# m4rch1n0/vqvae

Hardware: AMD Instinct MI355X
Metric: latents/sec through geodesic kNN+APSP+K-medoids (higher is better)
Workload: dtype f64-exact(u32 fixed point)

## Files before the change

include/geo_hip.h:

```cpp
#ifndef GEO_HIP_H
#define GEO_HIP_H

#include <stddef.h>
#include <stdint.h>

#ifdef __cplusplus
extern "C" {
#endif

#define GEO_OK 0
#define GEO_E_ARG (-1)
#define GEO_E_WORKSPACE (-2)
#define GEO_E_HIP (-3)
#define GEO_E_NOCONV (-4)

int geo_version(void);
const char *geo_last_error(void);

int geo_set_option(const char *name, int32_t value);

size_t geo_sssp_workspace_bytes(int32_t n, int64_t nnz, int32_t n_sources);

int geo_sssp_multi(const int32_t *indptr, const int32_t *indices, const float *weights,
                   int32_t n, int64_t nnz, const int32_t *sources, int32_t n_sources,
// ... 139 lines not shown
#define GEO_JVP_MID_PIPE 0
#define GEO_JVP_MID_PIPE_DEDUP 1
#define GEO_JVP_MID_ALL 2
#define GEO_JVP_MID_ALL_TANGENT 3
#define GEO_JVP_MID_CHUNK 4
#define GEO_JVP_BACK_MFMA 0
#define GEO_JVP_BACK_PER_NODE 1
#define GEO_JVP_BACK_DEDUP 2
#define GEO_JVP_BACK_VALU 3
#define GEO_JVP_PLAN_FRONT(p) ((p) & 3)
#define GEO_JVP_PLAN_DMAX(p) (16 << (((p) >> 2) & 3))
#define GEO_JVP_PLAN_MID(p) (((p) >> 4) & 15)
#define GEO_JVP_PLAN_BACK(p) (((p) >> 8) & 15)
#define GEO_JVP_PER_NODE 0x1000
#define GEO_JVP_NODE_JACOBIAN 0x2000
#define GEO_JVP_DEDUP 0x4000
#define GEO_JVP_FRONT_ONCE 0x8000
#define GEO_JVP_PLAN_PASSES(p) ((p) >> 16)
int geo_jvp_plan(const geo_decoder_desc *dec, int64_t n_nodes, int64_t n_edges, int32_t batch_size, int32_t graph_edges,
                 size_t ws_bytes);
int geo_jvp_plan_part(const geo_decoder_desc *dec, int64_t n_nodes, int64_t n_edges, int64_t build_edges, int32_t batch_size,
                      int32_t graph_edges, size_t ws_bytes);
int geo_jvp_head_stream(const geo_decoder_desc *dec, int64_t n_nodes, int64_t n_edges, int32_t batch_size, int32_t graph_edges);

int geo_decoder_jvp_pairs(const geo_decoder_desc *dec, const float *z_start, const float *z_end,
                          int64_t n_edges, int32_t batch_size, float *len_out,
                          void *ws, size_t ws_bytes, void *stream);


typedef struct geo_vanilla_decoder_desc {
    int32_t latent_dim;
    int32_t c1, c2;
    int32_t out_channels;
    int32_t out_size;
    const float *At;
    const float *c;
    const float *w2p;
    const float *scale2;
    const float *shift2;
    const float *w3p;
    const float *b3;
} geo_vanilla_decoder_desc;

size_t geo_vanilla_jvp_workspace_bytes(const geo_vanilla_decoder_desc *dec, int64_t n_edges);
size_t geo_vanilla_jvp_edges_workspace_bytes(const geo_vanilla_decoder_desc *dec, int64_t n_nodes, int64_t n_edges);
int geo_vanilla_jvp_pairs(const geo_vanilla_decoder_desc *dec, const float *z_start, const float *z_end, int64_t n_edges,
// ... 155 lines not shown
```

vqvae_amd/_lib.py:

```python
import ctypes
import os

import torch

_HERE = os.path.dirname(os.path.abspath(__file__))
LIB_PATH = os.path.join(_HERE, "libgeo_hip.so")

c_p = ctypes.c_void_p
i32, i64, sz = ctypes.c_int32, ctypes.c_int64, ctypes.c_size_t


class DecoderDesc(ctypes.Structure):
    _fields_ = ([(n, i32) for n in ("latent_dim", "c0", "c1", "c2", "out_channels", "out_size", "norm",
                                    "bn_train", "groups1", "groups2")]
                + [("eps", ctypes.c_float)]
                + [(n, c_p) for n in ("w_in", "b_in", "w1", "b1", "g1", "be1", "rm1", "rv1",
                                      "w2", "b2", "g2", "be2", "rm2", "rv2", "w3", "b3")]
                + [("update_running", i32), ("momentum", ctypes.c_float)])


class VanillaDecoderDesc(ctypes.Structure):
    _fields_ = ([(n, i32) for n in ("latent_dim", "c1", "c2", "out_channels", "out_size")]
                + [(n, c_p) for n in ("At", "c", "w2p", "scale2", "shift2", "w3p", "b3")])

# ... 55 lines not shown
    "geo_knn_last_path": (ctypes.c_int, []),
    "geo_knn_thresholds": (ctypes.c_int, [c_p, i64, i32, i32, i32, i64, i64, i32, c_p, c_p, sz, c_p]),
    "geo_nearest_foreign_workspace_bytes": (sz, [i64, i32]),
    "geo_nearest_foreign": (ctypes.c_int, [c_p, i64, i32, i32, c_p, c_p, i64, c_p, c_p, c_p, sz, c_p]),
    "geo_bridge_components_workspace_bytes": (sz, [i64, i32, i32]),
    "geo_bridge_components": (ctypes.c_int, [c_p, i64, i32, i32, c_p, i32, c_p, c_p, c_p, c_p, sz, c_p]),
    "geo_csr_insert_workspace_bytes": (sz, [i32, i64]),
    "geo_csr_insert_count": (ctypes.c_int, [c_p, c_p, i32, c_p, c_p, c_p, i64, c_p, c_p, c_p, sz, c_p]),
    "geo_csr_insert_fill": (ctypes.c_int, [c_p, c_p, c_p, i32, i64, c_p, c_p, c_p, c_p, sz, c_p]),
    "geo_symmetrize_workspace_bytes": (sz, [i32, i32]),
    "geo_symmetrize_count": (ctypes.c_int, [c_p, c_p, i32, i32, i32, c_p, c_p, c_p, sz, c_p]),
    "geo_symmetrize_fill": (ctypes.c_int, [c_p, c_p, i32, i32, i32, c_p, c_p, c_p, c_p, sz, c_p]),
    "geo_upper_edges_count": (ctypes.c_int, [c_p, c_p, i32, c_p, c_p, c_p, sz, c_p]),
    "geo_upper_edges_fill": (ctypes.c_int, [c_p, c_p, i32, c_p, c_p, c_p, c_p, c_p]),
    "geo_cc_workspace_bytes": (sz, [i32]),
    "geo_connected_components": (ctypes.c_int, [c_p, c_p, i32, c_p, c_p, c_p, sz, c_p]),
    "geo_csr_compact_workspace_bytes": (sz, [i32]),
    "geo_csr_compact_count": (ctypes.c_int, [c_p, c_p, c_p, i32, c_p, i32, c_p, c_p, c_p, c_p, c_p, sz, c_p]),
    "geo_csr_compact_fill": (ctypes.c_int, [c_p, c_p, c_p, i32, c_p, i32, c_p, c_p, c_p, c_p, c_p]),
    "geo_jvp_workspace_bytes": (sz, [ctypes.POINTER(DecoderDesc), i64, i32]),
    "geo_jvp_edges_workspace_bytes": (sz, [ctypes.POINTER(DecoderDesc), i64, i64, i32]),
    "geo_jvp_plan": (ctypes.c_int, [ctypes.POINTER(DecoderDesc), i64, i64, i32, i32, sz]),
    "geo_jvp_head_stream": (ctypes.c_int, [ctypes.POINTER(DecoderDesc), i64, i64, i32, i32]),
    "geo_decoder_jvp_edges": (ctypes.c_int, [ctypes.POINTER(DecoderDesc), c_p, i64, c_p, c_p, i64, i32, c_p, c_p, sz, c_p]),
    "geo_jvp_edges_part_workspace_bytes": (sz, [ctypes.POINTER(DecoderDesc), i64, i64, i64, i32]),
    "geo_jvp_plan_part": (ctypes.c_int, [ctypes.POINTER(DecoderDesc), i64, i64, i64, i32, i32, sz]),
    "geo_decoder_jvp_edges_part": (ctypes.c_int, [ctypes.POINTER(DecoderDesc), c_p, i64, c_p, c_p, i64, i64, i32, c_p, c_p, sz,
                                                  c_p]),
    "geo_decoder_jvp_pairs": (ctypes.c_int, [ctypes.POINTER(DecoderDesc), c_p, c_p, i64, i32, c_p, c_p, sz, c_p]),
    "geo_vanilla_jvp_workspace_bytes": (sz, [ctypes.POINTER(VanillaDecoderDesc), i64]),
    "geo_vanilla_jvp_edges_workspace_bytes": (sz, [ctypes.POINTER(VanillaDecoderDesc), i64, i64]),
    "geo_vanilla_jvp_pairs": (ctypes.c_int, [ctypes.POINTER(VanillaDecoderDesc), c_p, c_p, i64, i32, c_p, c_p, sz, c_p]),
    "geo_vanilla_jvp_edges": (ctypes.c_int, [ctypes.POINTER(VanillaDecoderDesc), c_p, i64, c_p, c_p, i64, i32, c_p, c_p, sz, c_p]),
    "geo_vanilla_decode_workspace_bytes": (sz, [ctypes.POINTER(VanillaDecoderDesc), i64]),
    "geo_vanilla_decode": (ctypes.c_int, [ctypes.POINTER(VanillaDecoderDesc), c_p, c_p, i64, c_p, c_p, sz, c_p]),
    "geo_spatial_decode_workspace_bytes": (sz, [ctypes.POINTER(SpatialImageDecoderDesc), i64]),
    "geo_spatial_decode": (ctypes.c_int, [ctypes.POINTER(SpatialImageDecoderDesc), c_p, c_p, c_p, i64, c_p, c_p, sz, c_p]),
    "geo_image_encode_workspace_bytes": (sz, [ctypes.POINTER(ImageEncoderDesc), i64]),
    "geo_image_encode": (ctypes.c_int, [ctypes.POINTER(ImageEncoderDesc), c_p, i64, c_p, c_p, c_p, sz, c_p]),
    "geo_lpips_alex_workspace_bytes": (sz, [i64]),
    "geo_lpips_alex": (ctypes.c_int, [ctypes.POINTER(LPIPSAlexDesc), c_p, c_p, i64, c_p, c_p, c_p, sz, c_p]),
    "geo_gather_edge_weights":(ctypes.c_int, [c_p, c_p, i64, c_p, c_p]),
    "geo_prior_sample_workspace_bytes": (sz, [ctypes.POINTER(PriorDesc), i32, i32]),
    "geo_prior_sample": (ctypes.c_int, [ctypes.POINTER(PriorDesc), c_p, i32, i32, c_p, c_p, ctypes.c_float, i32, c_p, c_p, i32,
                                        c_p, sz, c_p]),
    "geo_kmeans_workspace_bytes": (sz, [i64, i32, i32, i32, i32]),
# ... 67 lines not shown
```

vqvae_amd/csrc/common.hip:

```cpp
#include "geo_common.h"

#include <cstdlib>
#include <cstring>

namespace geo {

namespace {
struct OptionName { const char *name, *env; int Options::*field; };
const OptionName kOptionNames[] = {
    {"sssp_sb", "GEO_SSSP_SB", &Options::sssp_sb},
    {"sssp_act", "GEO_SSSP_ACT", &Options::sssp_act},
    {"sssp_sparse_div", "GEO_SSSP_SPARSE_DIV", &Options::sssp_sparse_div},
    {"sssp_map_div", "GEO_SSSP_MAP_DIV", &Options::sssp_map_div},
    {"sssp_group", "GEO_SSSP_GROUP", &Options::sssp_group},
    {"sssp_grouped_cap", "GEO_SSSP_GROUPED_CAP", &Options::sssp_grouped_cap},
    {"sssp_trace", "GEO_SSSP_TRACE", &Options::sssp_trace},
    {"sssp_u32", "GEO_SSSP_U32", &Options::sssp_u32},
    {"sssp_push", "GEO_SSSP_PUSH", &Options::sssp_push},
    {"sssp_order", "GEO_SSSP_ORDER", &Options::sssp_order},
    {"sssp_delta", "GEO_SSSP_DELTA", &Options::sssp_delta},
    {"sssp_push_blocks", "GEO_SSSP_PUSH_BLOCKS", &Options::sssp_push_blocks},
    {"knn_filter", "GEO_KNN_FILTER", &Options::knn_filter},
    {"kpp_grid", "GEO_KPP_GRID", &Options::kpp_grid},
    {"kpp_profile", "GEO_KPP_PROFILE", &Options::kpp_profile},
    {"jvp_mid", "GEO_JVP_MID", &Options::jvp_mid},
    {"jvp_back_valu", "GEO_JVP_BACK_VALU", &Options::jvp_back_valu},
    {"jvp_front_valu", "GEO_JVP_FRONT_VALU", &Options::jvp_front_valu},
    {"jvp_per_node", "GEO_JVP_PER_NODE", &Options::jvp_per_node},
    {"jvp_node_jacobian", "GEO_JVP_NODE_JACOBIAN", &Options::jvp_node_jacobian},
    {"jvp_start_dedup", "GEO_JVP_START_DEDUP", &Options::jvp_start_dedup},
    {"jvp_front_once", "GEO_JVP_FRONT_ONCE", &Options::jvp_front_once},
    {"jvp_head_stream", "GEO_JVP_HEAD_STREAM", &Options::jvp_head_stream},
};
Options from_environment() {
    Options o;
    for (const OptionName &e : kOptionNames) {
        const char *v = getenv(e.env);
        if (!v) continue;
        if (e.field == &Options::jvp_mid) o.jvp_mid = v[0] == 'c' ? 2 : (v[0] == 'a' ? 3 : atoi(v));
        else o.*(e.field) = atoi(v);
    }
    return o;
}
}

Options &options() {
    static Options o = from_environment();
    return o;
}

static thread_local char g_err[512] = "";

void set_error(const char *fmt, ...) {
    va_list ap;
    va_start(ap, fmt);
// ... 87 lines not shown
    int rc = scan_rec(sums, offs, t, ar, s);
    if (rc != GEO_OK) return rc;
    scan_add_kernel<<<dim3((unsigned)t), dim3(SCAN_THREADS), 0, s>>>(out, offs, n, t);
    GEO_LAUNCH_CHECK();
    return GEO_OK;
}

int exclusive_scan_i32(const int32_t *in, int32_t *out, int64_t n, void *tmp, size_t tmp_bytes,
                       int64_t *total_host, hipStream_t stream) {
    Arena ar(tmp, tmp_bytes);
    int rc = scan_rec(in, out, n, ar, stream);
    if (rc != GEO_OK) return rc;
    if (total_host) {
        int32_t tot = 0;
        GEO_HIP_CHECK(hipMemcpyAsync(&tot, out + n, sizeof(int32_t), hipMemcpyDeviceToHost, stream));
        GEO_HIP_CHECK(hipStreamSynchronize(stream));
        *total_host = tot;
    }
    return GEO_OK;
}

}

extern "C" int geo_version(void) { return 114; }
extern "C" const char *geo_last_error(void) { return geo::g_err; }

extern "C" int geo_set_option(const char *name, int32_t value) {
    if (name)
        for (const geo::OptionName &e : geo::kOptionNames)
            if (strcmp(name, e.name) == 0) {
                geo::options().*(e.field) = value;
                return GEO_OK;
            }
    geo::set_error("geo_set_option: unknown option '%s'", name ? name : "(null)");
    return GEO_E_ARG;
}
```

vqvae_amd/csrc/geo_common.h:

```cpp
#pragma once
#include <hip/hip_runtime.h>

#include <cstdarg>
#include <cstdint>
#include <cstdio>

#include "geo_hip.h"

namespace geo {

void set_error(const char *fmt, ...);

#define GEO_HIP_CHECK(expr)                                                                      \
    do {                                                                                         \
        hipError_t _e = (expr);                                                                  \
        if (_e != hipSuccess) {                                                                  \
            geo::set_error("%s failed: %s (%s:%d)", #expr, hipGetErrorString(_e), __FILE__, __LINE__); \
            return GEO_E_HIP;                                                                    \
        }                                                                                        \
    } while (0)

#define GEO_REQUIRE(cond, ...)              \
    do {                                    \
        if (!(cond)) {                      \
            geo::set_error(__VA_ARGS__);    \
            return GEO_E_ARG;               \
        }                                   \
    } while (0)

#define GEO_LAUNCH_CHECK() GEO_HIP_CHECK(hipGetLastError())

struct Options {
    int sssp_sb = -1, sssp_act = 1, sssp_sparse_div = -1, sssp_map_div = -1, sssp_group = 1, sssp_grouped_cap = 256,
        sssp_trace = 0, sssp_u32 = 1, sssp_push = 1 ,
        sssp_delta = 8 , sssp_order = 0 , sssp_push_blocks = 64, knn_filter = 1, kpp_grid = 256, kpp_profile = 0, jvp_mid = 0 ,
        jvp_back_valu = 0, jvp_front_valu = 0, jvp_per_node = 1 ,
        jvp_node_jacobian = 1 ,
        jvp_start_dedup = 1 ,
        jvp_front_once = 1 ,
        jvp_head_stream = 1 ;
};
Options &options();

static inline size_t align_up(size_t x, size_t a = 256) { return (x + a - 1) / a * a; }

struct Arena {
    char *base;
    size_t size, off;
    Arena(void *p, size_t n) : base(static_cast<char *>(p)), size(n), off(0) {}
    template <typename T>
    T *take(size_t count) {
        size_t bytes = align_up(count * sizeof(T));
        if (off + bytes > size) return nullptr;
        T *r = reinterpret_cast<T *>(base + off);
        off += bytes;
        return r;
    }
};

static inline int64_t shrink_pass(int64_t items) { return items > 64 ? items - items / 8 : items - 1; }

static inline size_t pass_bytes(const size_t *per_item, int nb, int64_t items) {
    size_t bytes = 0;
// ... 41 lines not shown
```

vqvae_amd/csrc/jvp.hip:

```cpp
#include "geo_common.h"

#include <cmath>
#include <cstdlib>
#include <type_traits>
#include <vector>

namespace {

constexpr int TS = 32;
constexpr int NC = 128;
constexpr int MAX_BLOCKS = 4;
constexpr int FRONT_MAX_N1 = 1024;
constexpr int BACK_TS = 8;

typedef float f32x16 __attribute__((ext_vector_type(16)));
typedef __bf16 bf16x8 __attribute__((ext_vector_type(8)));
typedef unsigned short u16x8 __attribute__((ext_vector_type(8)));

struct Shape {
    int d, c0, c1, c2, co, s_out, pad3, p_out;
    int n1, n2;
    int opix_per_chunk, n_chunks;
};

// ... 1136 lines not shown
        const int64_t e = e_base + (int64_t)chunk * batch + within;
        const bool valid = within < slots_per_group && within < batch && e < n_edges;
        const bool head = valid && start_run_head(src, e, within);
        const unsigned long long m = __ballot(head);
        const int below = __popcll(m & ((1ull << lane) - 1ull));
        if (lane == 0) wsum[wave] = __popcll(m);
        __syncthreads();
        int before = carry, total = carry;
        for (int w = 0; w < 4; ++w) { if (w < wave) before += wsum[w]; total += wsum[w]; }
        const int k = before + below + (head ? 1 : 0) - 1;
        if (within < slots_per_group) {
            row_map[g0 + within] = (int32_t)(g0 + (valid ? k : 0));
            if (head) rep[g0 + k] = (int32_t)(g0 + within);
        }
        carry = total;
        __syncthreads();
    }
    if (threadIdx.x == 0) { carry_s = carry; n_compact[chunk] = carry; }
    __syncthreads();
    const int cnt = carry_s, padded = (cnt + TS - 1) / TS * TS;
    for (int k = cnt + (int)threadIdx.x; k < padded; k += 256) rep[g0 + k] = (int32_t)g0;
}

template <bool TT, bool ONCE = false>
__global__ __launch_bounds__(512, 2) void mid_start_kernel(const float *__restrict__ pre1, const float *__restrict__ tpre1,
                                                          const NormConst *__restrict__ consts1, int tiles_per_group,
                                                          const unsigned short *__restrict__ B3, const float *__restrict__ b2,
                                                          float *__restrict__ pre2, float *__restrict__ tpre2,
                                                          double *__restrict__ partial2, const int32_t *__restrict__ row_map,
                                                          const int32_t *__restrict__ rep, const int32_t *__restrict__ n_compact,
                                                          int64_t e_base, int64_t n_edges, int batch) {
    constexpr int C1 = 128, LDK = C1 + 8, KS = C1 / 16, NL = 4, c2 = 64, n1 = 4 * C1, n2 = 16 * c2;
    typedef float f32x2 __attribute__((ext_vector_type(2)));
    __shared__ __attribute__((aligned(16))) unsigned short A3[2][3][2][TS][LDK];
    const int chunk = blockIdx.y, group = 2 * chunk;
    const int ncomp = TT ? 0 : n_compact[chunk];
    auto run = [&](int item) {
    const int lt0 = 2 * item;
    const bool live1 = TT ? lt0 + 1 < tiles_per_group : (lt0 + 1) * TS < ncomp;
    const int tile0 = group * tiles_per_group + lt0, tile1 = live1 ? tile0 + 1 : tile0;
    const int lane = threadIdx.x & 63, wave = __builtin_amdgcn_readfirstlane((int)(threadIdx.x >> 6));
    const int wq = wave & 3, wg = wave >> 2;
    const int r = lane & 31, h = lane >> 5;
    f32x16 accp[NL], acct[NL];
#pragma unroll
    for (int lc = 0; lc < NL; ++lc)
#pragma unroll
        for (int i = 0; i < 16; ++i) { accp[lc][i] = 0.f; acct[lc][i] = 0.f; }

    const int k0p = 2 * lane, s0p = 4 * wave;
    const NormConst *kp = consts1 + (size_t)group * C1 + k0p;
    const NormConst kA = kp[0], kB = kp[1];
    static_assert(TT || !ONCE, "ONCE selects where the tangent launch reads");
    size_t xrow[2][4];
    const size_t g0 = (size_t)group * tiles_per_group * TS, group_slots = (size_t)tiles_per_group * TS;
    unsigned xoff[2][4], toff[2];
    __amdgpu_buffer_rsrc_t x_src, t_src;
#pragma unroll
    for (int i = 0; i < 4; ++i) {
        const size_t s0 = (size_t)tile0 * TS + s0p + i, s1 = (size_t)tile1 * TS + s0p + i;
        if (ONCE) {
            xoff[0][i] = (unsigned)(__builtin_amdgcn_readfirstlane(rep[__builtin_amdgcn_readfirstlane(row_map[s0])]) - (int)g0) * (n1 * 4u);
            xoff[1][i] = (unsigned)(__builtin_amdgcn_readfirstlane(rep[__builtin_amdgcn_readfirstlane(row_map[s1])]) - (int)g0) * (n1 * 4u);
        } else {
            xrow[0][i] = TT ? s0 : (size_t)__builtin_amdgcn_readfirstlane(rep[s0]);
            xrow[1][i] = TT ? s1 : (size_t)__builtin_amdgcn_readfirstlane(rep[s1]);
        }
    }
    if (ONCE) {
        x_src = __builtin_amdgcn_make_buffer_rsrc(const_cast<float *>(pre1 + g0 * n1), 0, (int)(group_slots * n1 * 4), 0x00020000);
        t_src = __builtin_amdgcn_make_buffer_rsrc(const_cast<float *>(tpre1 + (g0 + group_slots) * n1), 0, (int)(group_slots * n1 * 4), 0x00020000);
        toff[0] = (unsigned)(lt0 * TS + s0p) * (n1 * 4u);
        toff[1] = (unsigned)((live1 ? lt0 + 1 : lt0) * TS + s0p) * (n1 * 4u);
    }
    const unsigned v_pair = (unsigned)k0p * 4u;
    f32x2 rx[2][4], rt[2][4];
    auto fetch = [&](int nx) {
#pragma unroll
        for (int hh = 0; hh < 2; ++hh)
#pragma unroll
            for (int i = 0; i < 4; ++i) {
                if (ONCE) {
                    const int px_off = MidGeom::pix(nx) * C1 * 4;
                    rx[hh][i] = __builtin_bit_cast(f32x2, __builtin_amdgcn_raw_buffer_load_b64(x_src, v_pair, xoff[hh][i] + px_off, 0));
                    rt[hh][i] = __builtin_bit_cast(f32x2, __builtin_amdgcn_raw_buffer_load_b64(t_src, v_pair, toff[hh] + i * n1 * 4 + px_off, 0));
                    continue;
                }
                const size_t off = xrow[hh][i] * n1 + (size_t)MidGeom::pix(nx) * C1 + k0p;
                rx[hh][i] = *reinterpret_cast<const f32x2 *>(pre1 + off);
                if (TT) rt[hh][i] = *reinterpret_cast<const f32x2 *>(tpre1 + off);
            }
    };
    fetch(0);
    auto stage_px = [&](int buf, int nx) {
#pragma unroll
        for (int hh = 0; hh < 2; ++hh)
#pragma unroll
            for (int i = 0; i < 4; ++i) {
                float a0, t0, a1, t1;
                norm_relu(kA, rx[hh][i].x, TT ? rt[hh][i].x : 0.f, &a0, &t0);
                norm_relu(kB, rx[hh][i].y, TT ? rt[hh][i].y : 0.f, &a1, &t1);
                unsigned w[3];
                if (TT) split3_pair(t0, t1, w[0], w[1], w[2]);
                else split3_pair(a0, a1, w[0], w[1], w[2]);
#pragma unroll
                for (int part = 0; part < 3; ++part) *reinterpret_cast<unsigned *>(&A3[buf][part][hh][s0p + i][k0p]) = w[part];
            }
        if (nx < 4) {
            fetch(nx);
            __builtin_amdgcn_sched_group_barrier(0x020, TT ? 16 : 8, 0);
        }
    };
    bf16x8 ring[3][3];
    const unsigned b_lane = (unsigned)(h * 3 * NC * 8 + (wq * 32 + r) * 8) * 2u;
    const __amdgpu_buffer_rsrc_t b_rsrc = __builtin_amdgcn_make_buffer_rsrc(
        const_cast<unsigned short *>(B3), 0, (int)((size_t)8 * MAX_BLOCKS * C1 * NC * 3 * 2), 0x00020000);
    {
        const int cb0 = wg == 0 ? MidGeom::prod_cb(0, MidGeom::pix(0), 0) : MidGeom::prod_cb(1, MidGeom::pix(0), 0);
        const int cb1 = wg == 0 ? MidGeom::prod_cb(0, MidGeom::pix(0), 1) : MidGeom::prod_cb(1, MidGeom::pix(0), 1);
#pragma unroll
        for (int part = 0; part < 3; ++part) {
            ring[0][part] = __builtin_bit_cast(bf16x8, __builtin_amdgcn_raw_buffer_load_b128(b_rsrc, b_lane, (cb0 * KS * 2 * 3 + part) * NC * 8 * 2, 0));
            ring[1][part] = __builtin_bit_cast(bf16x8, __builtin_amdgcn_raw_buffer_load_b128(b_rsrc, b_lane, (cb1 * KS * 2 * 3 + part) * NC * 8 * 2, 0));
        }
    }
    stage_px(0, 1);
    if (wg == 1) __builtin_amdgcn_s_setprio(1);
    lds_barrier();
    const unsigned short *a3 = &A3[0][0][0][0][0];
    const unsigned a_lane = (unsigned)(r * LDK + h * 8);
    constexpr unsigned A_BUF = 3u * 2u * TS * LDK;
#define GEO_MID_PIXEL(WGV, IPV) mid_products<C1, false, WGV, IPV>(a3, a_lane + ((IPV) & 1) * A_BUF, b_rsrc, b_lane, accp, acct, ring)
    if (wg == 0) {
        GEO_MID_PIXEL(0, 0); stage_px(1, 2); lds_barrier();
        GEO_MID_PIXEL(0, 1); stage_px(0, 3); lds_barrier();
        GEO_MID_PIXEL(0, 2); stage_px(1, 4); lds_barrier();
        GEO_MID_PIXEL(0, 3);
    } else {
        stage_px(1, 2); GEO_MID_PIXEL(1, 0); lds_barrier();
        stage_px(0, 3); GEO_MID_PIXEL(1, 1); lds_barrier();
        stage_px(1, 4); GEO_MID_PIXEL(1, 2); lds_barrier();
        GEO_MID_PIXEL(1, 3);
    }
#undef GEO_MID_PIXEL

    const int lo = wq >> 1, co = (wq & 1) * 32 + r;
    const float bias = TT ? 0.f : b2[co];
    float *dst = TT ? tpre2 : pre2;
#pragma unroll
    for (int hh = 0; hh < 2; ++hh) {
        if (hh == 1 && !live1) break;
        const size_t tbase = (size_t)(hh ? tile1 : tile0) * TS;
#pragma unroll
        for (int lc = 0; lc < NL; ++lc) {
            const int ch = wg == 0 ? MidGeom::chunk_of(0, lc) : MidGeom::chunk_of(1, lc);
            const int op = lo == 0 ? MidGeom::opix(ch, 0) : MidGeom::opix(ch, 1);
#pragma unroll
            for (int q = 0; q < 16; ++q) {
                const int row = (q & 3) + 8 * (q >> 2) + 4 * h;
                const float v = hh ? acct[lc][q] : accp[lc][q];
                dst[(tbase + row) * n2 + (size_t)op * c2 + co] = TT ? v : v + bias;
            }
        }
    }
    if (TT) {
        int64_t cnt_g = n_edges - (e_base + (int64_t)chunk * batch);
        if (cnt_g > batch) cnt_g = batch;
#pragma unroll
        for (int hh = 0; hh < 2; ++hh) {
            if (hh == 1 && !live1) break;
            const int tile = hh ? tile1 : tile0;
            const size_t tbase = (size_t)tile * TS;
            const int n_valid = (int)cnt_g - (tile - group * tiles_per_group) * TS;
            Bn2Sums sums;
#pragma unroll
            for (int lc = 0; lc < NL; ++lc) {
                const int ch = wg == 0 ? MidGeom::chunk_of(0, lc) : MidGeom::chunk_of(1, lc);
                const int op = lo == 0 ? MidGeom::opix(ch, 0) : MidGeom::opix(ch, 1);
#pragma unroll
                for (int q = 0; q < 16; ++q) {
                    const int row = (q & 3) + 8 * (q >> 2) + 4 * h;
                    const float x = pre2[(size_t)row_map[tbase + row] * n2 + (size_t)op * c2 + co];
                    bn2_add(sums, x, hh ? acct[lc][q] : accp[lc][q], row < n_valid);
                }
            }
            bn2_store(sums, partial2, tile, wg * 2 + (wq >> 1), co, lane);
        }
    }
    };
    if (TT) {
        run((int)blockIdx.x);
    } else {
        for (int item = 0; 2 * item * TS < ncomp; ++item) {
            if (item > 0) { __builtin_amdgcn_s_setprio(0); __syncthreads(); }
            run(item);
        }
    }
}

__global__ __launch_bounds__(256) void slot_valid_kernel(int64_t e_base, int64_t n_edges, int batch, int tiles_per_group,
                                                        int64_t n_slots, int32_t *__restrict__ slot_valid) {
    for (int64_t i = (int64_t)blockIdx.x * blockDim.x + threadIdx.x; i < n_slots; i += (int64_t)gridDim.x * blockDim.x) {
        const int64_t per_group = (int64_t)tiles_per_group * TS;
        const int64_t g = i / per_group, within = i % per_group;
        const int64_t e = e_base + (g >> 1) * batch + within;
        slot_valid[i] = (within < batch && e < n_edges) ? 1 : 0;
    }
}

__global__ __launch_bounds__(256) void slot_node_kernel(const int32_t *__restrict__ src, const int32_t *__restrict__ dst,
// ... 554 lines not shown
    b += geo::align_up(tiles * s.n1 * 4 * 8) + geo::align_up(tiles * s.n2 * 4 * 8);
    b += geo::align_up((groups + 1) * s.c1 * sizeof(NormConst)) + geo::align_up((groups + 1) * s.c2 * sizeof(NormConst));
    b += geo::align_up((groups + 1) * (size_t)(s.c1 > s.c2 ? s.c1 : s.c2) * sizeof(float2));
    b += geo::align_up(slots * 4) * 2;
    if (dc->norm == 2) b += 2 * geo::align_up(slots * 32 * sizeof(float4));
    p->bytes = b + 4096;
    return true;
}

enum { BACK_NODE_PRIMAL = 15 };

struct Route {
    int status = GEO_OK;
    char error[192] = "";
    Plan pl = {};
    int64_t run_edges = 0, passes = 0;
    bool batch_stats = false, track = false, group_norm = false;
    int front = GEO_JVP_FRONT_VALU, dmax = 16;
    int mid = GEO_JVP_MID_CHUNK, back = GEO_JVP_BACK_VALU;
    int back_nt = 0;
    int parts2 = 16;
    bool per_node = false, node_jacobian = false, dedup = false, front_once = false;
    bool head_stream = false;
    size_t back_lds = 0;
    size_t jac_np = 0, jac_extra_bytes = 0;
    size_t bytes = 0;
};

bool route_error(Route *r, int status, const char *fmt, ...) {
    va_list ap;
    va_start(ap, fmt);
    vsnprintf(r->error, sizeof(r->error), fmt, ap);
    va_end(ap);
    r->status = status;
    return false;
}

bool make_route(const geo_decoder_desc *dc, const geo::Options &o, bool graph_edges, int64_t n_nodes, int64_t n_edges,
                int64_t build_edges, int batch, const size_t *ws_bytes, Route *r) {
    *r = Route{};
    if (!dc) return route_error(r, GEO_E_ARG, "geo_decoder_jvp: null pointer");
    if (batch <= 0) return route_error(r, GEO_E_ARG, "geo_decoder_jvp: batch_size must be positive");
    if (build_edges < n_edges)
        return route_error(r, GEO_E_ARG, "geo_decoder_jvp: build_edges %lld < n_edges %lld", (long long)build_edges,
                           (long long)n_edges);
    Plan base;
// ... 31 lines not shown
    r->pl = r->node_jacobian ? jpl : base;
    r->run_edges = r->node_jacobian ? n_pseudo : n_edges;
    const int64_t chunks = (r->run_edges + batch - 1) / batch;
    r->passes = (chunks + r->pl.chunks_per_pass - 1) / r->pl.chunks_per_pass;
    const size_t run_ws = ws - (r->node_jacobian ? r->jac_extra_bytes : 0);
    r->per_node = per_node_kernels && node_slots && node_slots <= r->pl.pass_slots() &&
                  run_ws >= r->pl.bytes + node_bytes(s, n_nodes);
    const size_t slots = r->pl.pass_slots(), tiles = slots / TS, groups = (size_t)r->pl.chunks_per_pass * 2;
    r->dedup = r->batch_stats && graph_edges && mid_pipe && back_mfma && o.jvp_start_dedup != 0 &&
               (2 * slots + groups) * 4 <= tiles * s.n1 * 4 * 8 && (size_t)r->back_nt * 32 <= (size_t)s.n1;
    r->front_once = r->dedup && r->front == GEO_JVP_FRONT_VALU && o.jvp_front_once != 0 && s.n1 == FRONT_EDGE_N1 &&
                    tiles * s.c1 * 4 * 8 + (2 * slots + groups) * 4 <= tiles * s.n1 * 4 * 8 &&
                    (size_t)base.slots_per_group * s.n1 * 4 < ((size_t)1 << 31);

    r->mid = r->per_node ? GEO_JVP_MID_ALL_TANGENT
           : mid_pipe    ? (r->dedup ? GEO_JVP_MID_PIPE_DEDUP : GEO_JVP_MID_PIPE)
           : mid_all     ? GEO_JVP_MID_ALL
                         : GEO_JVP_MID_CHUNK;
    r->parts2 = mid_pipe && !r->per_node ? 4 : (mid_all ? 1 : 16);
    r->back = r->dedup ? GEO_JVP_BACK_DEDUP : r->per_node ? GEO_JVP_BACK_PER_NODE : back_mfma ? GEO_JVP_BACK_MFMA : GEO_JVP_BACK_VALU;
    r->head_stream = back_mfma && r->back_nt == 1 && !r->group_norm && (r->back == GEO_JVP_BACK_DEDUP || r->back == GEO_JVP_BACK_MFMA) &&
                     o.jvp_head_stream != 0 &&
                     (!r->dedup || (size_t)base.slots_per_group * s.n2 * 4 < ((size_t)1 << 31));
    r->back_lds = ((size_t)2 * BACK_TS * 16 * (s.c2 + 4) + (size_t)16 * s.co * (s.c2 + 4) + (size_t)BACK_TS * s.p_out) * 4;

    if (!(s.d >= 1 && s.d <= 64)) return route_error(r, GEO_E_ARG, "geo_decoder_jvp: latent_dim %d not in [1,64]", s.d);
    if (!(s.c1 == 128 || s.c1 == 64 || s.c1 == 32))
        return route_error(r, GEO_E_ARG, "geo_decoder_jvp: dec_channels[1]=%d not in {32,64,128}", s.c1);
    if (!(dc->norm >= 0 && dc->norm <= 2)) return route_error(r, GEO_E_ARG, "geo_decoder_jvp: unknown norm code %d", dc->norm);
    if (s.c2 % 16 != 0) return route_error(r, GEO_E_ARG, "geo_decoder_jvp: dec_channels[2]=%d must be a multiple of 16", s.c2);
    if (r->back_lds > 160 * 1024)
        return route_error(r, GEO_E_ARG, "geo_decoder_jvp: decoder too wide for the back kernel (%zu B LDS)", r->back_lds);
    if (run_ws < r->pl.bytes) return route_error(r, GEO_E_WORKSPACE, "geo_decoder_jvp: workspace %zu < %zu", run_ws, r->pl.bytes);
    if (r->group_norm && !(dc->groups1 == 32 && dc->groups2 == 32 && s.c2 == 64 && back_mfma && mid_all))
        return route_error(r, GEO_E_ARG,
                           "geo_decoder_jvp: GroupNorm needs 32 groups per layer and dec_channels[2] == 64 (got %d/%d groups, c2=%d)",
                           dc->groups1, dc->groups2, s.c2);
    return true;
}

int encode_route(const Route &r) {
    const int64_t passes = r.passes < 0x7fff ? r.passes : 0x7fff;
    return r.front | (r.dmax == 16 ? 0 : (r.dmax == 32 ? 1 : 2)) << 2 | r.mid << 4 | r.back << 8 |
           (r.per_node ? GEO_JVP_PER_NODE : 0) | (r.node_jacobian ? GEO_JVP_NODE_JACOBIAN : 0) | (r.dedup ? GEO_JVP_DEDUP : 0) |
           (r.front_once ? GEO_JVP_FRONT_ONCE : 0) | (int)passes << 16;
}
// ... 101 lines not shown
int launch_mid(const Route &r, const geo_decoder_desc *dc, const Pass &p, const Buffers &b, hipStream_t stream) {
    const Shape &s = r.pl.sh;
    if (p.mid == GEO_JVP_MID_PIPE || p.mid == GEO_JVP_MID_PIPE_DEDUP) {
        const bool dedup = p.mid == GEO_JVP_MID_PIPE_DEDUP;
        const int64_t chunks = p.groups() / 2;
        if (dedup && !r.front_once)
            if (const int rc = launch_start_runs(p, b, stream)) return rc;
        int n_cu = 0;
        if (const int rc = cu_count(&n_cu)) return rc;
        const int64_t pipe_tiles = dedup ? p.tiles / 2 : p.tiles;
        const unsigned grid = (unsigned)std::min<int64_t>(pipe_tiles, n_cu);
        pick_bool(dedup, [&](auto end_only) {
            mid_pipe_kernel<decltype(end_only)::value><<<grid, 512, 0, stream>>>(
                b.pre1, b.tpre1, b.k1, p.stat, p.tiles_per_group, (int)pipe_tiles, s.c2, b.B3, dc->b2, p.mid_pre2, b.tpre2, b.part2,
                p.stat, p.e_base, p.n_edges, p.batch);
        });
        GEO_LAUNCH_CHECK();
        if (dedup) {
            mid_start_kernel<false><<<dim3(1, (unsigned)chunks), 512, 0, stream>>>(
                b.pre1, b.tpre1, b.k1, p.tiles_per_group, b.B3, dc->b2, p.mid_pre2, b.tpre2, b.part2, b.row_map, b.rep, b.n_compact,
                p.e_base, p.n_edges, p.batch);
            GEO_LAUNCH_CHECK();
            pick_bool(r.front_once, [&](auto once) {
                mid_start_kernel<true, decltype(once)::value>
                    <<<dim3((unsigned)((p.tiles_per_group + 1) / 2), (unsigned)chunks), 512, 0, stream>>>(
                        b.pre1, b.tpre1, b.k1, p.tiles_per_group, b.B3, dc->b2, p.mid_pre2, b.tpre2, b.part2, b.row_map, b.rep,
                        b.n_compact, p.e_base, p.n_edges, p.batch);
            });
            GEO_LAUNCH_CHECK();
        }
    } else if (p.mid == GEO_JVP_MID_ALL || p.mid == GEO_JVP_MID_ALL_TANGENT) {
        pick_int<128, 64, 32>(s.c1, [&](auto c1) {
            pick_bool(r.group_norm, [&](auto gn) {
                pick_bool(p.mid == GEO_JVP_MID_ALL_TANGENT, [&](auto tangent_only) {
                    mid_all_kernel<decltype(c1)::value, decltype(gn)::value, decltype(tangent_only)::value>
                        <<<(unsigned)p.tiles, 512, 0, stream>>>(b.pre1, b.tpre1, b.k1, p.stat, p.tiles_per_group, s.c2, b.B3, dc->b2,
                                                                p.mid_pre2, b.tpre2, b.part2, p.stat, b.slot_valid, b.gs1, p.e_base,
                                                                p.n_edges, p.batch);
                });
            });
        });
        GEO_LAUNCH_CHECK();
    } else {
        pick_int<128, 64, 32>(s.c1, [&](auto c1) {
            mid_bf16_kernel<decltype(c1)::value><<<dim3((unsigned)p.tiles, (unsigned)s.n_chunks), 256, 0, stream>>>(
                b.pre1, b.tpre1, b.k1, p.stat, p.tiles_per_group, b.tab, s.opix_per_chunk, s.c2, b.B3, dc->b2, p.mid_pre2, b.tpre2,
                b.part2, p.stat, b.slot_valid);
        });
        GEO_LAUNCH_CHECK();
    }
// ... 181 lines not shown
}

int decoder_jvp(const geo_decoder_desc *dc, const geo::Options &opt, bool graph_edges, const float *z, int64_t n_nodes,
                const int32_t *src, const int32_t *dst, const float *z_start, const float *z_end, int64_t n_edges,
                int64_t build_edges, int32_t batch, float *len_out, void *ws, size_t ws_bytes, void *stream) {
    GEO_REQUIRE(dc && len_out && ws, "geo_decoder_jvp: null pointer");
    GEO_REQUIRE(batch > 0, "geo_decoder_jvp: batch_size must be positive");
    if (n_edges == 0) return GEO_OK;
    Route r;
    if (!make_route(dc, opt, graph_edges, n_nodes, n_edges, build_edges, batch, &ws_bytes, &r)) {
        geo::set_error("%s", r.error);
        return r.status;
    }
    return run_jvp(dc, r, z, n_nodes, src, dst, z_start, z_end, n_edges, len_out, ws, ws_bytes, static_cast<hipStream_t>(stream));
}

}

#ifdef GEO_MID_PROF
extern "C" int geo_debug_mid_prof(unsigned long long *out, int reset) {
    if (reset) { unsigned long long z[16] = {0}; return (int)hipMemcpyToSymbol(HIP_SYMBOL(g_mid_prof), z, sizeof(z)); }
    return (int)hipMemcpyFromSymbol(out, HIP_SYMBOL(g_mid_prof), sizeof(unsigned long long) * 16);
}
#endif

extern "C" size_t geo_jvp_workspace_bytes(const geo_decoder_desc *dec, int64_t n_edges, int32_t batch_size) {
    const geo::Options opt = geo::options();
    Route r;
    make_route(dec, opt, false, 0, n_edges, n_edges, batch_size, nullptr, &r);
    return r.bytes;
}

extern "C" size_t geo_jvp_edges_part_workspace_bytes(const geo_decoder_desc *dec, int64_t n_nodes, int64_t n_edges,
                                                     int64_t build_edges, int32_t batch_size) {
    const geo::Options opt = geo::options();
    Route r;
    make_route(dec, opt, true, n_nodes, n_edges, build_edges, batch_size, nullptr, &r);
    return r.bytes;
}

extern "C" size_t geo_jvp_edges_workspace_bytes(const geo_decoder_desc *dec, int64_t n_nodes, int64_t n_edges,
                                                int32_t batch_size) {
    return geo_jvp_edges_part_workspace_bytes(dec, n_nodes, n_edges, n_edges, batch_size);
}

extern "C" int geo_jvp_plan_part(const geo_decoder_desc *dec, int64_t n_nodes, int64_t n_edges, int64_t build_edges,
                                 int32_t batch_size, int32_t graph_edges, size_t ws_bytes) {
    const geo::Options opt = geo::options();
    Route r;
    if (!make_route(dec, opt, graph_edges != 0, graph_edges ? n_nodes : 0, n_edges, build_edges, batch_size,
                    ws_bytes ? &ws_bytes : nullptr, &r)) {
        geo::set_error("%s", r.error);
        return r.status;
    }
    return encode_route(r);
}

extern "C" int geo_jvp_plan(const geo_decoder_desc *dec, int64_t n_nodes, int64_t n_edges, int32_t batch_size,
                            int32_t graph_edges, size_t ws_bytes) {
    return geo_jvp_plan_part(dec, n_nodes, n_edges, n_edges, batch_size, graph_edges, ws_bytes);
}

extern "C" int geo_jvp_head_stream(const geo_decoder_desc *dec, int64_t n_nodes, int64_t n_edges, int32_t batch_size,
                                   int32_t graph_edges) {
    const geo::Options opt = geo::options();
    Route r;
    if (!make_route(dec, opt, graph_edges != 0, graph_edges ? n_nodes : 0, n_edges, n_edges, batch_size, nullptr, &r)) {
        geo::set_error("%s", r.error);
        return r.status;
    }
    return r.head_stream ? 1 : 0;
}

extern "C" int geo_decoder_jvp_edges_part(const geo_decoder_desc *dec, const float *z, int64_t n_nodes, const int32_t *src,
                                          const int32_t *dst, int64_t n_edges, int64_t build_edges, int32_t batch_size,
                                          float *len_out, void *ws, size_t ws_bytes, void *stream) {
    GEO_REQUIRE(build_edges >= n_edges, "geo_decoder_jvp_edges_part: build_edges %lld < n_edges %lld", (long long)build_edges,
                (long long)n_edges);
    GEO_REQUIRE(n_edges == 0 || (z && src && dst && n_nodes > 0), "geo_decoder_jvp_edges: null pointer");
    const geo::Options opt = geo::options();
    return decoder_jvp(dec, opt, true, z, n_nodes, src, dst, nullptr, nullptr, n_edges, build_edges, batch_size, len_out, ws,
                       ws_bytes, stream);
}

// ... 15 lines not shown
```

Measured before the change: 2.559 million.

## Stage compact primal rows in LDS for mid_start tangent BN2 reduction

In the tangent mid_start kernel with dedup, the few compact pre2 rows that a tile pair references are prefetched with buffer loads during the last pixel stage and copied into the freed A3 LDS buffer, so the BN2 statistics read them from LDS instead of gathering from global memory through row_map. It also splits the pre1 fetch and staging into halves to lower register pressure, and switches output stores to buffer stores with precomputed offsets. The path adds an extra barrier and only applies when the rows fit the fixed limit, otherwise it falls back to the global gather. Optional profiling stamps are compiled in only under a debug macro.

Result: slower. 2.520 million (-1.5%).

```diff
diff --git a/include/geo_hip.h b/include/geo_hip.h
--- a/include/geo_hip.h
+++ b/include/geo_hip.h
@@ -185,6 +185,7 @@
 int geo_jvp_plan_part(const geo_decoder_desc *dec, int64_t n_nodes, int64_t n_edges, int64_t build_edges, int32_t batch_size,
                       int32_t graph_edges, size_t ws_bytes);
 int geo_jvp_head_stream(const geo_decoder_desc *dec, int64_t n_nodes, int64_t n_edges, int32_t batch_size, int32_t graph_edges);
+int geo_jvp_mid_start_lds_rows(void);
 
 int geo_decoder_jvp_pairs(const geo_decoder_desc *dec, const float *z_start, const float *z_end,
                           int64_t n_edges, int32_t batch_size, float *len_out,
diff --git a/vqvae_amd/_lib.py b/vqvae_amd/_lib.py
--- a/vqvae_amd/_lib.py
+++ b/vqvae_amd/_lib.py
@@ -101,6 +101,7 @@
     "geo_jvp_edges_workspace_bytes": (sz, [ctypes.POINTER(DecoderDesc), i64, i64, i32]),
     "geo_jvp_plan": (ctypes.c_int, [ctypes.POINTER(DecoderDesc), i64, i64, i32, i32, sz]),
     "geo_jvp_head_stream": (ctypes.c_int, [ctypes.POINTER(DecoderDesc), i64, i64, i32, i32]),
+    "geo_jvp_mid_start_lds_rows": (ctypes.c_int, []),
     "geo_decoder_jvp_edges": (ctypes.c_int, [ctypes.POINTER(DecoderDesc), c_p, i64, c_p, c_p, i64, i32, c_p, c_p, sz, c_p]),
     "geo_jvp_edges_part_workspace_bytes": (sz, [ctypes.POINTER(DecoderDesc), i64, i64, i64, i32]),
     "geo_jvp_plan_part": (ctypes.c_int, [ctypes.POINTER(DecoderDesc), i64, i64, i64, i32, i32, sz]),
diff --git a/vqvae_amd/csrc/common.hip b/vqvae_amd/csrc/common.hip
--- a/vqvae_amd/csrc/common.hip
+++ b/vqvae_amd/csrc/common.hip
@@ -31,6 +31,7 @@
     {"jvp_start_dedup", "GEO_JVP_START_DEDUP", &Options::jvp_start_dedup},
     {"jvp_front_once", "GEO_JVP_FRONT_ONCE", &Options::jvp_front_once},
     {"jvp_head_stream", "GEO_JVP_HEAD_STREAM", &Options::jvp_head_stream},
+    {"jvp_mid_start_lds", "GEO_JVP_MID_START_LDS", &Options::jvp_mid_start_lds},
 };
 Options from_environment() {
     Options o;
@@ -164,7 +165,7 @@
 
 }
 
-extern "C" int geo_version(void) { return 114; }
+extern "C" int geo_version(void) { return 115; }
 extern "C" const char *geo_last_error(void) { return geo::g_err; }
 
 extern "C" int geo_set_option(const char *name, int32_t value) {
diff --git a/vqvae_amd/csrc/geo_common.h b/vqvae_amd/csrc/geo_common.h
--- a/vqvae_amd/csrc/geo_common.h
+++ b/vqvae_amd/csrc/geo_common.h
@@ -38,7 +38,8 @@
         jvp_node_jacobian = 1 ,
         jvp_start_dedup = 1 ,
         jvp_front_once = 1 ,
-        jvp_head_stream = 1 ;
+        jvp_head_stream = 1 ,
+        jvp_mid_start_lds = 1 ;
 };
 Options &options();
 
diff --git a/vqvae_amd/csrc/jvp.hip b/vqvae_amd/csrc/jvp.hip
--- a/vqvae_amd/csrc/jvp.hip
+++ b/vqvae_amd/csrc/jvp.hip
@@ -1182,7 +1182,22 @@
     for (int k = cnt + (int)threadIdx.x; k < padded; k += 256) rep[g0 + k] = (int32_t)g0;
 }
 
-template <bool TT, bool ONCE = false>
+constexpr int MID_START_LDS_ROWS = 12;
+#ifdef GEO_MID_PROF
+__device__ unsigned long long g_start_prof[2][10];
+#define GEO_SP_STAMP(slot)                                                                                             \
+    do { if (TT && ONCE) { const unsigned long long t_ = __builtin_amdgcn_s_memtime();                                  \
+                           if (lane == 0 && wq == 0) atomicAdd(&g_start_prof[wg][slot], t_ - sp_prev);                  \
+                           sp_prev = t_; } } while (0)
+#define GEO_SP_BARRIER(slot) do { GEO_SP_STAMP(slot); lds_barrier(); GEO_SP_STAMP(5); } while (0)
+#else
+#define GEO_SP_STAMP(slot)
+#define GEO_SP_BARRIER(slot) lds_barrier()
+#endif
+static_assert((size_t)MID_START_LDS_ROWS * 16 * 64 * sizeof(float) <= (size_t)3 * 2 * TS * (128 + 8) * sizeof(unsigned short),
+              "the copied compact rows must fit one A3 buffer");
+static_assert(MID_START_LDS_ROWS % 2 == 0 && MID_START_LDS_ROWS * 256 % 512 == 0, "whole 16-byte loads per thread");
+template <bool TT, bool ONCE = false, bool XLDS = false>
 __global__ __launch_bounds__(512, 2) void mid_start_kernel(const float *__restrict__ pre1, const float *__restrict__ tpre1,
                                                           const NormConst *__restrict__ consts1, int tiles_per_group,
                                                           const unsigned short *__restrict__ B3, const float *__restrict__ b2,
@@ -1193,6 +1208,8 @@
     constexpr int C1 = 128, LDK = C1 + 8, KS = C1 / 16, NL = 4, c2 = 64, n1 = 4 * C1, n2 = 16 * c2;
     typedef float f32x2 __attribute__((ext_vector_type(2)));
     __shared__ __attribute__((aligned(16))) unsigned short A3[2][3][2][TS][LDK];
+    __shared__ int x_row[2 * TS];
+    static_assert(TT || !XLDS, "XLDS selects where the tangent launch reads its primal");
     const int chunk = blockIdx.y, group = 2 * chunk;
     const int ncomp = TT ? 0 : n_compact[chunk];
     auto run = [&](int item) {
@@ -1202,6 +1219,24 @@
     const int lane = threadIdx.x & 63, wave = __builtin_amdgcn_readfirstlane((int)(threadIdx.x >> 6));
     const int wq = wave & 3, wg = wave >> 2;
     const int r = lane & 31, h = lane >> 5;
+#ifdef GEO_MID_PROF
+    unsigned long long sp_prev = __builtin_amdgcn_s_memtime();
+#endif
+    int64_t cnt_g = n_edges - (e_base + (int64_t)chunk * batch);
+    if (cnt_g > batch) cnt_g = batch;
+    int x_first = 0, x_rows = 0;
+    if (XLDS) {
+        int nv = (int)cnt_g - lt0 * TS;
+        nv = nv < 1 ? 1 : (nv > (live1 ? 2 * TS : TS) ? (live1 ? 2 * TS : TS) : nv);
+        x_first = __builtin_amdgcn_readfirstlane(row_map[(size_t)tile0 * TS]);
+        x_rows = __builtin_amdgcn_readfirstlane(row_map[(size_t)tile0 * TS + nv - 1]) - x_first + 1;
+        if (x_rows < 1 || x_rows > MID_START_LDS_ROWS) x_rows = 0;
+        if (x_rows && threadIdx.x < 2 * TS) {
+            int loc = row_map[(size_t)(threadIdx.x < TS ? tile0 : tile1) * TS + (threadIdx.x & (TS - 1))] - x_first;
+            loc = loc < 0 ? 0 : (loc >= x_rows ? x_rows - 1 : loc);
+            x_row[threadIdx.x] = loc * n2;
+        }
+    }
     f32x16 accp[NL], acct[NL];
 #pragma unroll
     for (int lc = 0; lc < NL; ++lc)
@@ -1234,42 +1269,45 @@
         toff[1] = (unsigned)((live1 ? lt0 + 1 : lt0) * TS + s0p) * (n1 * 4u);
     }
     const unsigned v_pair = (unsigned)k0p * 4u;
-    f32x2 rx[2][4], rt[2][4];
-    auto fetch = [&](int nx) {
-#pragma unroll
-        for (int hh = 0; hh < 2; ++hh)
-#pragma unroll
-            for (int i = 0; i < 4; ++i) {
-                if (ONCE) {
-                    const int px_off = MidGeom::pix(nx) * C1 * 4;
-                    rx[hh][i] = __builtin_bit_cast(f32x2, __builtin_amdgcn_raw_buffer_load_b64(x_src, v_pair, xoff[hh][i] + px_off, 0));
-                    rt[hh][i] = __builtin_bit_cast(f32x2, __builtin_amdgcn_raw_buffer_load_b64(t_src, v_pair, toff[hh] + i * n1 * 4 + px_off, 0));
-                    continue;
-                }
-                const size_t off = xrow[hh][i] * n1 + (size_t)MidGeom::pix(nx) * C1 + k0p;
-                rx[hh][i] = *reinterpret_cast<const f32x2 *>(pre1 + off);
-                if (TT) rt[hh][i] = *reinterpret_cast<const f32x2 *>(tpre1 + off);
-            }
+    f32x2 rx[4], rt[4];
+    auto fetch = [&](int nx, int hh) {
+#pragma unroll
+        for (int i = 0; i < 4; ++i) {
+            if (ONCE) {
+                const int px_off = MidGeom::pix(nx) * C1 * 4;
+                rx[i] = __builtin_bit_cast(f32x2, __builtin_amdgcn_raw_buffer_load_b64(x_src, v_pair, xoff[hh][i] + px_off, 0));
+                rt[i] = __builtin_bit_cast(f32x2, __builtin_amdgcn_raw_buffer_load_b64(t_src, v_pair, toff[hh] + i * n1 * 4 + px_off, 0));
+                continue;
+            }
+            const size_t off = xrow[hh][i] * n1 + (size_t)MidGeom::pix(nx) * C1 + k0p;
+            rx[i] = *reinterpret_cast<const f32x2 *>(pre1 + off);
+            if (TT) rt[i] = *reinterpret_cast<const f32x2 *>(tpre1 + off);
+        }
+        __builtin_amdgcn_sched_group_barrier(0x020, TT ? 8 : 4, 0);
     };
-    fetch(0);
+    fetch(0, 0);
+    auto stage_half = [&](int buf, int hh) {
+        unsigned w_idx = (unsigned)(((buf * 3 * 2 + hh) * TS + s0p) * LDK + k0p);
+        asm volatile("" : "+v"(w_idx));
+        unsigned short *w3 = &A3[0][0][0][0][0] + w_idx;
+#pragma unroll
+        for (int i = 0; i < 4; ++i) {
+            float a0, t0, a1, t1;
+            norm_relu(kA, rx[i].x, TT ? rt[i].x : 0.f, &a0, &t0);
+            norm_relu(kB, rx[i].y, TT ? rt[i].y : 0.f, &a1, &t1);
+            unsigned w[3];
+            if (TT) split3_pair(t0, t1, w[0], w[1], w[2]);
+            else split3_pair(a0, a1, w[0], w[1], w[2]);
+#pragma unroll
+            for (int part = 0; part < 3; ++part) *reinterpret_cast<unsigned *>(w3 + part * 2 * TS * LDK + i * LDK) = w[part];
+        }
+    };
     auto stage_px = [&](int buf, int nx) {
-#pragma unroll
-        for (int hh = 0; hh < 2; ++hh)
-#pragma unroll
-            for (int i = 0; i < 4; ++i) {
-                float a0, t0, a1, t1;
-                norm_relu(kA, rx[hh][i].x, TT ? rt[hh][i].x : 0.f, &a0, &t0);
-                norm_relu(kB, rx[hh][i].y, TT ? rt[hh][i].y : 0.f, &a1, &t1);
-                unsigned w[3];
-                if (TT) split3_pair(t0, t1, w[0], w[1], w[2]);
-                else split3_pair(a0, a1, w[0], w[1], w[2]);
-#pragma unroll
-                for (int part = 0; part < 3; ++part) *reinterpret_cast<unsigned *>(&A3[buf][part][hh][s0p + i][k0p]) = w[part];
-            }
-        if (nx < 4) {
-            fetch(nx);
-            __builtin_amdgcn_sched_group_barrier(0x020, TT ? 16 : 8, 0);
-        }
+        stage_half(buf, 0);
+        fetch(nx - 1, 1);
+        __builtin_amdgcn_sched_barrier(0);
+        stage_half(buf, 1);
+        if (nx < 4) fetch(nx, 0);
     };
     bf16x8 ring[3][3];
     const unsigned b_lane = (unsigned)(h * 3 * NC * 8 + (wq * 32 + r) * 8) * 2u;
@@ -1286,66 +1324,103 @@
     }
     stage_px(0, 1);
     if (wg == 1) __builtin_amdgcn_s_setprio(1);
-    lds_barrier();
+    GEO_SP_BARRIER(0);
     const unsigned short *a3 = &A3[0][0][0][0][0];
     const unsigned a_lane = (unsigned)(r * LDK + h * 8);
     constexpr unsigned A_BUF = 3u * 2u * TS * LDK;
 #define GEO_MID_PIXEL(WGV, IPV) mid_products<C1, false, WGV, IPV>(a3, a_lane + ((IPV) & 1) * A_BUF, b_rsrc, b_lane, accp, acct, ring)
+    constexpr int XJ = MID_START_LDS_ROWS / 2;
+    typedef float f32x4 __attribute__((ext_vector_type(4)));
+    f32x4 xc[XJ];
+    auto x_fetch = [&]() {
+        if (!XLDS || !x_rows) return;
+        const __amdgpu_buffer_rsrc_t x_cp = __builtin_amdgcn_make_buffer_rsrc(
+            const_cast<float *>(pre2 + (size_t)x_first * n2), 0, x_rows * n2 * 4, 0x00020000);
+#pragma unroll
+        for (int j = 0; j < XJ; ++j)
+            if (2 * j < x_rows)
+                xc[j] = __builtin_bit_cast(f32x4, __builtin_amdgcn_raw_buffer_load_b128(x_cp, (unsigned)threadIdx.x * 16u, j * 2 * n2 * 4, 0));
+    };
+    auto x_put = [&]() {
+        if (!XLDS || !x_rows) return;
+        f32x4 *xl = reinterpret_cast<f32x4 *>(&A3[0][0][0][0][0]);
+#pragma unroll
+        for (int j = 0; j < XJ; ++j)
+            if (2 * j < x_rows) xl[j * 512 + (int)threadIdx.x] = xc[j];
+    };
     if (wg == 0) {
-        GEO_MID_PIXEL(0, 0); stage_px(1, 2); lds_barrier();
-        GEO_MID_PIXEL(0, 1); stage_px(0, 3); lds_barrier();
-        GEO_MID_PIXEL(0, 2); stage_px(1, 4); lds_barrier();
-        GEO_MID_PIXEL(0, 3);
+        GEO_MID_PIXEL(0, 0); stage_px(1, 2); GEO_SP_BARRIER(1);
+        GEO_MID_PIXEL(0, 1); stage_px(0, 3); GEO_SP_BARRIER(2);
+        GEO_MID_PIXEL(0, 2); stage_px(1, 4); x_fetch(); GEO_SP_BARRIER(3);
+        x_put(); GEO_MID_PIXEL(0, 3);
     } else {
-        stage_px(1, 2); GEO_MID_PIXEL(1, 0); lds_barrier();
-        stage_px(0, 3); GEO_MID_PIXEL(1, 1); lds_barrier();
-        stage_px(1, 4); GEO_MID_PIXEL(1, 2); lds_barrier();
-        GEO_MID_PIXEL(1, 3);
-    }
+        stage_px(1, 2); GEO_MID_PIXEL(1, 0); GEO_SP_BARRIER(1);
+        stage_px(0, 3); GEO_MID_PIXEL(1, 1); GEO_SP_BARRIER(2);
+        stage_px(1, 4); GEO_MID_PIXEL(1, 2); x_fetch(); GEO_SP_BARRIER(3);
+        x_put(); GEO_MID_PIXEL(1, 3);
+    }
+    GEO_SP_STAMP(4);
+    if (XLDS && x_rows) GEO_SP_BARRIER(4);
 #undef GEO_MID_PIXEL
 
     const int lo = wq >> 1, co = (wq & 1) * 32 + r;
     const float bias = TT ? 0.f : b2[co];
     float *dst = TT ? tpre2 : pre2;
+    unsigned v_out = (unsigned)(4 * h * n2 + co) * 4u;
+    asm volatile("" : "+v"(v_out));
 #pragma unroll
     for (int hh = 0; hh < 2; ++hh) {
         if (hh == 1 && !live1) break;
         const size_t tbase = (size_t)(hh ? tile1 : tile0) * TS;
+        const __amdgpu_buffer_rsrc_t o_dst = __builtin_amdgcn_make_buffer_rsrc(dst + tbase * n2, 0, TS * n2 * 4, 0x00020000);
 #pragma unroll
         for (int lc = 0; lc < NL; ++lc) {
             const int ch = wg == 0 ? MidGeom::chunk_of(0, lc) : MidGeom::chunk_of(1, lc);
             const int op = lo == 0 ? MidGeom::opix(ch, 0) : MidGeom::opix(ch, 1);
 #pragma unroll
             for (int q = 0; q < 16; ++q) {
-                const int row = (q & 3) + 8 * (q >> 2) + 4 * h;
                 const float v = hh ? acct[lc][q] : accp[lc][q];
-                dst[(tbase + row) * n2 + (size_t)op * c2 + co] = TT ? v : v + bias;
-            }
-        }
-    }
+                const int soff = (((q & 3) + 8 * (q >> 2)) * n2 + op * c2) * 4;
+                __builtin_amdgcn_raw_buffer_store_b32(__float_as_uint(TT ? v : v + bias), o_dst, v_out, soff, 0);
+            }
+        }
+    }
+    GEO_SP_STAMP(6);
     if (TT) {
-        int64_t cnt_g = n_edges - (e_base + (int64_t)chunk * batch);
-        if (cnt_g > batch) cnt_g = batch;
-#pragma unroll
-        for (int hh = 0; hh < 2; ++hh) {
-            if (hh == 1 && !live1) break;
-            const int tile = hh ? tile1 : tile0;
-            const size_t tbase = (size_t)tile * TS;
-            const int n_valid = (int)cnt_g - (tile - group * tiles_per_group) * TS;
-            Bn2Sums sums;
-#pragma unroll
-            for (int lc = 0; lc < NL; ++lc) {
-                const int ch = wg == 0 ? MidGeom::chunk_of(0, lc) : MidGeom::chunk_of(1, lc);
-                const int op = lo == 0 ? MidGeom::opix(ch, 0) : MidGeom::opix(ch, 1);
-#pragma unroll
-                for (int q = 0; q < 16; ++q) {
-                    const int row = (q & 3) + 8 * (q >> 2) + 4 * h;
-                    const float x = pre2[(size_t)row_map[tbase + row] * n2 + (size_t)op * c2 + co];
-                    bn2_add(sums, x, hh ? acct[lc][q] : accp[lc][q], row < n_valid);
+        const float *xl = reinterpret_cast<const float *>(&A3[0][0][0][0][0]);
+        const bool from_lds = XLDS && x_rows;
+        {
+#pragma unroll
+            for (int hh = 0; hh < 2; ++hh) {
+                if (hh == 1 && !live1) break;
+                const int tile = hh ? tile1 : tile0;
+                const size_t tbase = (size_t)tile * TS;
+                const int n_valid = (int)cnt_g - (tile - group * tiles_per_group) * TS;
+                Bn2Sums sums;
+#pragma unroll
+                for (int lc = 0; lc < NL; ++lc) {
+                    const int ch = wg == 0 ? MidGeom::chunk_of(0, lc) : MidGeom::chunk_of(1, lc);
+                    const int op = lo == 0 ? MidGeom::opix(ch, 0) : MidGeom::opix(ch, 1);
+                    float x[16];
+                    if (from_lds) {
+#pragma unroll
+                        for (int q = 0; q < 16; ++q) x[q] = xl[x_row[hh * TS + (q & 3) + 8 * (q >> 2) + 4 * h] + op * c2 + co];
+                    } else {
+#pragma unroll
+                        for (int q = 0; q < 16; ++q)
+                            x[q] = pre2[(size_t)row_map[tbase + (q & 3) + 8 * (q >> 2) + 4 * h] * n2 + (size_t)op * c2 + co];
+                    }
+#pragma unroll
+                    for (int q = 0; q < 16; ++q)
+                        bn2_add(sums, x[q], hh ? acct[lc][q] : accp[lc][q], (q & 3) + 8 * (q >> 2) + 4 * h < n_valid);
                 }
-            }
-            bn2_store(sums, partial2, tile, wg * 2 + (wq >> 1), co, lane);
-        }
+                bn2_store(sums, partial2, tile, wg * 2 + (wq >> 1), co, lane);
+            }
+        }
+        GEO_SP_STAMP(7);
+#ifdef GEO_MID_PROF
+        if (ONCE && lane == 0 && wq == 0) atomicAdd(&g_start_prof[wg][8], 1ull);
+#endif
     }
     };
     if (TT) {
@@ -1946,6 +2021,7 @@
     int parts2 = 16;
     bool per_node = false, node_jacobian = false, dedup = false, front_once = false;
     bool head_stream = false;
+    bool mid_start_lds = false;
     size_t back_lds = 0;
     size_t jac_np = 0, jac_extra_bytes = 0;
     size_t bytes = 0;
@@ -2023,6 +2099,7 @@
     r->head_stream = back_mfma && r->back_nt == 1 && !r->group_norm && (r->back == GEO_JVP_BACK_DEDUP || r->back == GEO_JVP_BACK_MFMA) &&
                      o.jvp_head_stream != 0 &&
                      (!r->dedup || (size_t)base.slots_per_group * s.n2 * 4 < ((size_t)1 << 31));
+    r->mid_start_lds = r->dedup && o.jvp_mid_start_lds != 0;
     r->back_lds = ((size_t)2 * BACK_TS * 16 * (s.c2 + 4) + (size_t)16 * s.co * (s.c2 + 4) + (size_t)BACK_TS * s.p_out) * 4;
 
     if (!(s.d >= 1 && s.d <= 64)) return route_error(r, GEO_E_ARG, "geo_decoder_jvp: latent_dim %d not in [1,64]", s.d);
@@ -2170,10 +2247,12 @@
                 p.e_base, p.n_edges, p.batch);
             GEO_LAUNCH_CHECK();
             pick_bool(r.front_once, [&](auto once) {
-                mid_start_kernel<true, decltype(once)::value>
-                    <<<dim3((unsigned)((p.tiles_per_group + 1) / 2), (unsigned)chunks), 512, 0, stream>>>(
-                        b.pre1, b.tpre1, b.k1, p.tiles_per_group, b.B3, dc->b2, p.mid_pre2, b.tpre2, b.part2, b.row_map, b.rep,
-                        b.n_compact, p.e_base, p.n_edges, p.batch);
+                pick_bool(r.mid_start_lds, [&](auto xlds) {
+                    mid_start_kernel<true, decltype(once)::value, decltype(xlds)::value>
+                        <<<dim3((unsigned)((p.tiles_per_group + 1) / 2), (unsigned)chunks), 512, 0, stream>>>(
+                            b.pre1, b.tpre1, b.k1, p.tiles_per_group, b.B3, dc->b2, p.mid_pre2, b.tpre2, b.part2, b.row_map, b.rep,
+                            b.n_compact, p.e_base, p.n_edges, p.batch);
+                });
             });
             GEO_LAUNCH_CHECK();
         }
@@ -2401,6 +2480,10 @@
     if (reset) { unsigned long long z[16] = {0}; return (int)hipMemcpyToSymbol(HIP_SYMBOL(g_mid_prof), z, sizeof(z)); }
     return (int)hipMemcpyFromSymbol(out, HIP_SYMBOL(g_mid_prof), sizeof(unsigned long long) * 16);
 }
+extern "C" int geo_debug_mid_start_prof(unsigned long long *out, int reset) {
+    if (reset) { unsigned long long z[20] = {0}; return (int)hipMemcpyToSymbol(HIP_SYMBOL(g_start_prof), z, sizeof(z)); }
+    return (int)hipMemcpyFromSymbol(out, HIP_SYMBOL(g_start_prof), sizeof(unsigned long long) * 20);
+}
 #endif
 
 extern "C" size_t geo_jvp_workspace_bytes(const geo_decoder_desc *dec, int64_t n_edges, int32_t batch_size) {
@@ -2439,6 +2522,8 @@
                             int32_t graph_edges, size_t ws_bytes) {
     return geo_jvp_plan_part(dec, n_nodes, n_edges, n_edges, batch_size, graph_edges, ws_bytes);
 }
+
+extern "C" int geo_jvp_mid_start_lds_rows(void) { return geo::options().jvp_mid_start_lds != 0 ? MID_START_LDS_ROWS : 0; }
 
 extern "C" int geo_jvp_head_stream(const geo_decoder_desc *dec, int64_t n_nodes, int64_t n_edges, int32_t batch_size,
                                    int32_t graph_edges) {
```
